# camillabelponer/dealii-slod

Measured on AMD Instinct MI355X. Metric: SLOD patches/sec (basis built), 2D Poisson H=1/32 n_sub=8 oversampling 2, higher is better.
Workload: dtype f64; 1 GPU; C2: 2D Poisson SLOD, H=1/32, n_sub=8, oversampling=2, D1e4 coefficient (contrast 10000), 1024 patches on rank 0 (ensemble of 1 realisations, contiguous patch blocks); patches_per_gpu=1024, parallelism=patch-sharded x1

## Files before the change

dealii-slod_amd/csrc/slod_api.cpp:

```cpp
#include "slod_host.h"

#include <algorithm>
#include <cmath>
#include <cstdio>
#include <cstdlib>
#include <cstring>
#include <string>
#include <vector>

namespace
{
  struct PatchGeom
  {
    int cx, cy, x0, y0, mx, my;
    int side_domain[4];
  };
}

std::string &slod_create_error()
{
  static thread_local std::string e;
  return e;
}

struct slod_plan
{
  slod_handle               *h = nullptr;
  size_t                     n = 0;
  std::vector<SlodPatchDesc> desc;
  SlodPatchDesc             *d_desc = nullptr;
  SlodPatchDesc             *d_desc_bal = nullptr;
  int                        m_max = 0, L_max = 0, nc_max = 0, nb_max = 0, nn_max = 0, nf_max = 0;
  int                        nb_buf = 0;
  size_t                     stride = 0, out_size = 0;
  size_t                     chunk = 0;
  double                    *ws_st = nullptr, *ws_v = nullptr, *ws_x = nullptr, *ws_m = nullptr;
  double                    *ws_z = nullptr;
  double                    *ws_x_alloc = nullptr;
  size_t                     guard = 0;
  size_t                     st_stride = 0, v_stride = 0, x_stride = 0;
  int32_t                   *d_status = nullptr;
  SlodPatchDiag             *d_pdiag  = nullptr;
  SlodSolveChoice            choice;
  std::vector<hipEvent_t>    ev;
  size_t                     n_chunks = 0;
  int                        depth = 1;
  size_t                     n_exec = 0;
  bool                       ran = false;
  struct AltWs
  {
    double  *ws_st = nullptr, *ws_v = nullptr, *ws_x_alloc = nullptr, *ws_x = nullptr, *ws_z = nullptr, *ws_m = nullptr;
    int32_t *d_status = nullptr;
  } alt;
  int         overlap = 1;
  hipStream_t istream[2] = {nullptr, nullptr};
  hipEvent_t  fork_ev = nullptr, done_ev[2] = {nullptr, nullptr};
  bool        inflight[2] = {false, false};
  bool                       uniform_stride = true;
  std::vector<char>          prob_used;
// ... 122 lines not shown
    a.coef_stride = (size_t)h->NE * h->NE * 4;
    a.NE          = h->NE;
    a.n_sub       = h->cfg.n_subdivisions;
    a.quirk       = h->cfg.projection_quirk;
#ifdef SLOD_ENABLE_DIAG
    if (const char *dg = std::getenv("SLOD_DIAG"))
      a.diag = std::atoi(dg);
#endif
    const double H = 1.0 / (double)h->N, hh = H / (double)h->cfg.n_subdivisions;
    a.scale     = hh * hh / 4.0;
    a.invH2     = 1.0 / (H * H);
    a.st        = p->ws_st;
    a.st_stride = p->st_stride;
    a.nn_max    = p->nn_max;
    a.vinv      = p->ws_v;
    a.v_stride  = p->v_stride;
    a.m_max     = p->m_max;
    a.L_max     = p->L_max;
    a.xs        = p->ws_x;
    a.zs        = p->ws_z ? p->ws_z : p->ws_x;
    a.x_stride  = p->x_stride;
    a.nc_max    = p->nc_max;
    a.ms        = p->ws_m;
    a.m_fused   = 0;
    a.nb_buf    = p->nb_buf;
    a.nf_max    = p->nf_max;
    a.fuse_select = 0;
    a.fuse_assemble = 0;
    a.basis     = d_basis;
    a.premult   = d_premult;
    a.status    = p->d_status;
    a.pdiag     = p->d_pdiag;
    if (slot == 1)
      {
        a.st     = p->alt.ws_st;
        a.vinv   = p->alt.ws_v;
        a.xs     = p->alt.ws_x;
        a.zs     = p->alt.ws_z ? p->alt.ws_z : p->alt.ws_x;
        a.ms     = p->alt.ws_m;
        a.status = p->alt.d_status;
      }
    return a;
  }
}

namespace
{
  hipError_t launch_range(slod_plan *p, size_t first, int cnt, double *d_basis, double *d_premult, hipStream_t st,
                          hipEvent_t *ev, bool balanced, int slot = 0)
  {
    const int      s = p->h->cfg.spacedim;
    SlodKernelArgs a = make_args(p, first, d_basis, d_premult, balanced, slot);
    hipError_t     e = ev ? hipEventRecord(ev[0], st) : hipSuccess;
    if (e == hipSuccess && !p->choice.fuse_assemble)
      e = slod_launch_assemble(s, a, cnt, st);
    if (e == hipSuccess && ev)
      e = hipEventRecord(ev[1], st);
    if (e == hipSuccess)
      e = slod_launch_solve(s, p->choice, a, cnt, st);
    if (e == hipSuccess && ev)
      e = hipEventRecord(ev[2], st);
    if (e == hipSuccess && !a.fuse_select)
// ... 273 lines not shown
      return fail(h, SLOD_ERR_UNSUPPORTED, "slod_plan_create: more than 112 dofs per grid line");
    }
  if (p->nc_max > 64)
    {
      slod_plan_destroy(p);
      return fail(h, SLOD_ERR_UNSUPPORTED, "slod_plan_create: more than 64 coarse dofs per patch");
    }
  p->nb_buf = std::min(p->nb_max, std::max(s == 1 ? 96 : 80, p->nc_max + 16));
  if (p->nb_buf > 160)
    {
      slod_plan_destroy(p);
      return fail(h, SLOD_ERR_UNSUPPORTED, "slod_plan_create: boundary-trace buffer beyond the selection kernel's 160 rows");
    }
  if (!slod_choose_solver(s, n_sub, p->m_max, p->L_max, p->nc_max, p->nb_buf, p->nf_max, n, slod_read_tuning(), &p->choice))
    {
      slod_plan_destroy(p);
      return fail(h, SLOD_ERR_UNSUPPORTED, "slod_plan_create: patch does not fit the 160 KB LDS of any solver kernel");
    }
  p->nn_max    = (p->nn_max + 31) & ~31;
  p->st_stride = (size_t)9 * s * s * p->nn_max;
  p->v_stride  = p->choice.v_patch_elems ? p->choice.v_patch_elems : (size_t)p->L_max * p->choice.v_line_elems;
  p->x_stride  = (size_t)p->L_max * p->m_max * p->nc_max;
  const bool   own_z = p->choice.kind == SLOD_K_TW;
  const size_t per_patch = (p->st_stride + p->v_stride + (own_z ? 2 : 1) * p->x_stride) * sizeof(double);
  size_t budget_mb = 24 * 1024;
  {
    size_t free_b = 0, total_b = 0;
    if (hipMemGetInfo(&free_b, &total_b) == hipSuccess)
      {
        const size_t free_mb = free_b / (1024 * 1024);
        budget_mb = std::min(std::max<size_t>(budget_mb, free_mb * 6 / 10), std::max<size_t>(64, free_mb * 8 / 10));
      }
  }
  if (const char *env = std::getenv("SLOD_WORKSPACE_MB"))
    budget_mb = (size_t)std::max(1L, std::atol(env));
  p->chunk = std::max<size_t>(1, std::min<size_t>(n, budget_mb * 1024 * 1024 / per_patch));
  ok = true;
  p->guard = (size_t)24 * p->nc_max + 64;
  const size_t st_slack = (size_t)4 * p->nn_max;
  auto free_ws = [&]() {
    for (double **q : {&p->ws_st, &p->ws_v, &p->ws_x_alloc, &p->ws_z, &p->ws_m})
      if (*q)
        {
          (void)hipFree(*q);
          *q = nullptr;
        }
    p->ws_x = nullptr;
  };
  for (;;)
    {
      bool w = ok;
      w      = w && hipMalloc((void **)&p->ws_st, (p->chunk * p->st_stride + st_slack) * sizeof(double)) == hipSuccess;
      w      = w && hipMalloc((void **)&p->ws_v, std::max<size_t>(1, p->chunk * p->v_stride) * sizeof(double)) == hipSuccess;
      w      = w && hipMalloc((void **)&p->ws_x_alloc, (p->chunk * p->x_stride + 2 * p->guard) * sizeof(double)) == hipSuccess;
      if (own_z)
        w = w && hipMalloc((void **)&p->ws_z, (p->chunk * p->x_stride + p->guard) * sizeof(double)) == hipSuccess;
      w = w && hipMalloc((void **)&p->ws_m, p->chunk * (size_t)p->nc_max * p->nc_max * sizeof(double)) == hipSuccess;
      if (w || !ok || p->chunk == 1)
        {
          ok = w;
          break;
        }
      (void)hipGetLastError();
      free_ws();
      p->chunk = (p->chunk + 1) / 2;
    }
  ok      = ok && hipMemset(p->ws_st, 0, (p->chunk * p->st_stride + st_slack) * sizeof(double)) == hipSuccess;
  ok      = ok && hipMemset(p->ws_x_alloc, 0, (p->chunk * p->x_stride + 2 * p->guard) * sizeof(double)) == hipSuccess;
  p->ws_x = p->ws_x_alloc ? p->ws_x_alloc + p->guard : nullptr;
  if (own_z)
    ok = ok && hipMemset(p->ws_z, 0, (p->chunk * p->x_stride + p->guard) * sizeof(double)) == hipSuccess;
  ok       = ok && hipMalloc((void **)&p->d_status, sizeof(int32_t)) == hipSuccess;
  ok       = ok && hipMalloc((void **)&p->d_pdiag, n * (size_t)s * sizeof(SlodPatchDiag)) == hipSuccess;
  ok       = ok && hipMemset(p->d_pdiag, 0, n * (size_t)s * sizeof(SlodPatchDiag)) == hipSuccess;
  ok = ok && hipMemset(p->d_status, 0, sizeof(int32_t)) == hipSuccess;
  p->n_chunks = (n + p->chunk - 1) / p->chunk;
  p->ev.assign(4 * p->n_chunks, nullptr);
  for (auto &ev : p->ev)
    ok = ok && hipEventCreate(&ev) == hipSuccess;
  if (!ok)
// ... 102 lines not shown
    return SLOD_ERR_ARGUMENT;
  slod_handle *h = p->h;
  if (p->n == 0 || depth == p->overlap)
    return SLOD_OK;
  (void)hipSetDevice(h->cfg.device);
  (void)hipDeviceSynchronize();
  if (depth == 1)
    {
      p->overlap = 1;
      return SLOD_OK;
    }
  if (p->n_chunks != 1)
    return fail(h, SLOD_ERR_STATE, "slod_plan_set_overlap: the plan runs in several workspace chunks (they de-phase by themselves)");
  const bool own_z = p->ws_z != nullptr;
  const size_t st_slack = (size_t)4 * p->nn_max;
  bool ok = true;
  if (!p->alt.ws_st)
    {
      ok = ok && hipMalloc((void **)&p->alt.ws_st, (p->chunk * p->st_stride + st_slack) * sizeof(double)) == hipSuccess;
      ok = ok && hipMalloc((void **)&p->alt.ws_v, std::max<size_t>(1, p->chunk * p->v_stride) * sizeof(double)) == hipSuccess;
      ok = ok && hipMalloc((void **)&p->alt.ws_x_alloc, (p->chunk * p->x_stride + 2 * p->guard) * sizeof(double)) == hipSuccess;
      if (own_z)
        ok = ok && hipMalloc((void **)&p->alt.ws_z, (p->chunk * p->x_stride + p->guard) * sizeof(double)) == hipSuccess;
      ok = ok && hipMalloc((void **)&p->alt.ws_m, p->chunk * (size_t)p->nc_max * p->nc_max * sizeof(double)) == hipSuccess;
      ok = ok && hipMalloc((void **)&p->alt.d_status, sizeof(int32_t)) == hipSuccess;
      ok = ok && hipMemset(p->alt.ws_st, 0, (p->chunk * p->st_stride + st_slack) * sizeof(double)) == hipSuccess;
      ok = ok && hipMemset(p->alt.ws_x_alloc, 0, (p->chunk * p->x_stride + 2 * p->guard) * sizeof(double)) == hipSuccess;
      if (own_z)
        ok = ok && hipMemset(p->alt.ws_z, 0, (p->chunk * p->x_stride + p->guard) * sizeof(double)) == hipSuccess;
      ok = ok && hipMemset(p->alt.d_status, 0, sizeof(int32_t)) == hipSuccess;
      p->alt.ws_x = p->alt.ws_x_alloc ? p->alt.ws_x_alloc + p->guard : nullptr;
      for (int k = 0; k < 2 && ok; ++k)
        {
          ok = ok && hipStreamCreateWithFlags(&p->istream[k], hipStreamNonBlocking) == hipSuccess;
          ok = ok && hipEventCreateWithFlags(&p->done_ev[k], hipEventDisableTiming) == hipSuccess;
        }
      ok = ok && hipEventCreateWithFlags(&p->fork_ev, hipEventDisableTiming) == hipSuccess;
    }
  if (!ok)
    return hip_fail(h, hipGetLastError(), "slod_plan_set_overlap: device allocation");
  p->overlap = 2;
  p->n_exec  = 0;
  return SLOD_OK;
}

int slod_plan_join(slod_plan *p, void *hip_stream)
{
// ... 502 lines not shown
```

dealii-slod_amd/csrc/slod_device.h:

```cpp
#ifndef SLOD_DEVICE_H
#define SLOD_DEVICE_H

#include <hip/hip_runtime.h>
#include <stddef.h>
#include <stdint.h>

struct SlodPatchDesc
{
  int32_t  ox, oy;
  int32_t  nx, ny;
  int32_t  mx, my;
  int32_t  ccx, ccy;
  int32_t  flags;
  int32_t  m, L;
  int32_t  n_c, n_b;
  int32_t  prob;
  uint32_t plan_index;
  uint64_t out_off;
};

enum : int32_t
{
  SLOD_F_LOD        = 1 << 4,
  SLOD_F_TRANSPOSED = 1 << 5
};

#ifdef SLOD_ENABLE_DIAG
#define SLOD_DG(A, mask) ((A).diag & (mask))
#else
#define SLOD_DG(A, mask) 0
#endif

struct SlodPatchDiag
{
  int32_t path;
  int32_t n_cut;
  int32_t n_dropped;
  int32_t sweeps;
  double  dinf;
  double  sigma_max, sigma_min;
};

// ... 4 lines not shown
  const double        *coef1;
  size_t               coef_stride;
  int32_t              NE;
  int32_t              n_sub;
  int32_t              quirk;
  int32_t              diag;
  int32_t              debug;
  double               scale;
  double               invH2;
  double *st;
  size_t  st_stride;
  int32_t nn_max;
  double *vinv;
  size_t  v_stride;
  int32_t m_max;
  int32_t L_max;
  int32_t nv;
  double *xs;
  double *zs;
  size_t  x_stride;
  int32_t nc_max;
  double *ms;
  int32_t m_fused;
  int32_t nb_buf;
  int32_t nf_max;
  int32_t fuse_select;
  int32_t fuse_assemble;
  double  *basis;
  double  *premult;
  int32_t *status;
  SlodPatchDiag *pdiag;
};

enum SlodSolverKind : int32_t
{
  SLOD_K_MF   = 1,
  SLOD_K_TW   = 2,
  SLOD_K_WS   = 3,
  SLOD_K_COOP = 4,
  SLOD_K_ND   = 5
};

struct SlodTuning
{
  int solver = 0;
  int fuse_select = 1, fuse_assemble = 1, fuse_m = 0;
  int twisted = -1;
  int balance = 1;
  int debug = 0;
};
struct SlodSolveChoice
{
  int    kind = 0;
  size_t lds  = 0;
  int    fuse_select = 0, fuse_assemble = 0, m_fused = 0, twisted = 0, debug = 0;
  int    v_line_pad = 0;
  size_t v_line_elems = 0;
  int    nv = 0;
  size_t v_patch_elems = 0;
};
SlodTuning slod_read_tuning();
bool       slod_choose_solver(int S, int n_sub, int m_max, int L_max, int nc_max, int nb_buf, int nf_max, size_t n_patches,
                              const SlodTuning &t, SlodSolveChoice *out);

hipError_t slod_launch_assemble(int S, const SlodKernelArgs &a, int n_patches, hipStream_t st);
hipError_t slod_launch_solve(int S, const SlodSolveChoice &c, SlodKernelArgs &a, int n_patches, hipStream_t st);
hipError_t slod_launch_solve_mf(int S, const SlodKernelArgs &a, int n_patches, size_t lds, hipStream_t st);
hipError_t slod_launch_solve_tw(int S, const SlodKernelArgs &a, int n_patches, size_t lds, hipStream_t st);
hipError_t slod_launch_solve_ws(int S, const SlodKernelArgs &a, int n_patches, size_t lds, hipStream_t st);
hipError_t slod_launch_solve_coop(int S, int twisted, const SlodKernelArgs &a, int n_patches, hipStream_t st);
hipError_t slod_launch_solve_nd(const SlodKernelArgs &a, int n_patches, size_t lds, hipStream_t st);
int        slod_solve_nd_cell(int S, int n_sub, int m_max, int L_max);
size_t     slod_solve_nd_scratch(int nv, int m_max, int L_max, int nc_max);
size_t     slod_solve_nd_lds_bytes(int nv, int m_max, int nc_max);
hipError_t slod_launch_select(int S, const SlodKernelArgs &a, int n_patches, int nb_max,
                              int nf_max, hipStream_t st);
size_t     slod_solve_lds_bytes(int S, int m_max, int nc_max, int twisted);
size_t     slod_solve_ws_lds_bytes(int S, int m_max, int nc_max);
size_t     slod_solve_tw_lds_bytes(int S, int m_max, int nc_max);
size_t     slod_solve_mf_lds_bytes(int S, int m_max, int nc_max);
int        slod_solve_ws_tile(int m_max);
int        slod_solve_mf_tiles(int S, int m_max);
size_t     slod_select_lds_bytes(int S, int nb_max, int nc_max, int nf_max);

#endif
```

dealii-slod_amd/csrc/slod_dispatch.cpp:

```cpp
#include "slod_device.h"

#include <cstdlib>
#include <cstring>

SlodTuning slod_read_tuning()
{
  SlodTuning t;
  if (const char *sel = getenv("SLOD_SOLVE"))
    t.solver = !strcmp(sel, "mf") ? SLOD_K_MF : !strcmp(sel, "tw") ? SLOD_K_TW : !strcmp(sel, "ws") ? SLOD_K_WS :
               !strcmp(sel, "coop") ? SLOD_K_COOP : !strcmp(sel, "nd") ? SLOD_K_ND : 0;
  if (const char *e = getenv("SLOD_FUSE_SELECT"))
    t.fuse_select = atoi(e) ? 1 : 0;
  if (const char *e = getenv("SLOD_FUSE_ASSEMBLE"))
    t.fuse_assemble = atoi(e) ? 1 : 0;
  if (const char *e = getenv("SLOD_FUSE_M"))
    t.fuse_m = atoi(e) ? 1 : 0;
  if (const char *e = getenv("SLOD_TWISTED"))
    t.twisted = atoi(e) ? 1 : 0;
  if (const char *e = getenv("SLOD_BALANCE"))
    t.balance = atoi(e) ? 1 : 0;
  if (const char *e = getenv("SLOD_DEBUG"))
    t.debug = atoi(e) ? 1 : 0;
  return t;
}
// ... 22 lines not shown
      c.v_patch_elems = slod_solve_nd_scratch(nd_nv, m_max, L_max, nc_max);
      c.fuse_assemble = t.fuse_assemble ? 1 : 0;
      c.fuse_select   = 0;
    }
  else if (mf_fits && (t.solver == SLOD_K_MF || (t.solver == 0 && !tw_fits && !ws_fits)))
    {
      c.kind          = SLOD_K_MF;
      c.lds           = slod_solve_mf_lds_bytes(S, m_max, nc_max);
      c.v_line_pad    = 16 * slod_solve_mf_tiles(S, m_max);
      c.v_line_elems  = (size_t)c.v_line_pad * c.v_line_pad;
      c.fuse_assemble = (S == 1 && t.fuse_assemble) ? 1 : 0;
      c.fuse_select   = (S == 1 && t.fuse_select && lds_sel <= lds_max) ? 1 : 0;
      if (c.fuse_select && lds_sel > c.lds)
        c.lds = lds_sel;
    }
  else if (want(SLOD_K_TW) && tw_fits)
    {
      c.kind          = SLOD_K_TW;
      c.lds           = slod_solve_tw_lds_bytes(S, m_max, nc_max);
      c.v_line_pad    = 8 * wt;
      c.v_line_elems  = (size_t)64 * wt * wt;
      c.fuse_assemble = (S == 1 && t.fuse_assemble) ? 1 : 0;
      c.fuse_select = (S == 1 && t.fuse_select && lds_sel <= 64 * 1024) ? 1 : 0;
      if (c.fuse_select && lds_sel > c.lds)
        c.lds = lds_sel;
    }
  else if ((want(SLOD_K_WS) || t.solver == SLOD_K_TW) && ws_fits &&
           slod_solve_ws_lds_bytes(S, m_max, nc_max) <= lds_max)
    {
      c.kind       = SLOD_K_WS;
      c.lds        = slod_solve_ws_lds_bytes(S, m_max, nc_max);
      c.v_line_pad = 8 * wt;
      c.v_line_elems = (size_t)c.v_line_pad * c.v_line_pad;
      c.m_fused = (t.fuse_m && nc_max * nc_max <= 192 * 4) ? 1 : 0;
    }
  else if (t.solver == 0 || t.solver == SLOD_K_COOP || !ws_fits)
    {
      int tw = t.twisted >= 0 ? t.twisted : (n_patches < 3 * 256 ? 1 : 0);
      if (slod_solve_lds_bytes(S, m_max, nc_max, tw) > lds_max)
        tw = 0;
      if (slod_solve_lds_bytes(S, m_max, nc_max, tw) > lds_max || (m_max + 15) / 16 > 7)
        return false;
      c.kind       = SLOD_K_COOP;
      c.twisted    = tw;
      c.lds        = slod_solve_lds_bytes(S, m_max, nc_max, tw);
      c.v_line_pad = m_max;
      c.v_line_elems = (size_t)m_max * m_max;
    }
  else
    return false;
  if (!c.fuse_select && lds_sel > lds_max)
    return false;
  *out = c;
  return true;
}

hipError_t slod_launch_solve(int S, const SlodSolveChoice &c, SlodKernelArgs &a, int n_patches, hipStream_t st)
{
  a.m_fused       = c.m_fused;
  a.fuse_select   = c.fuse_select;
  a.fuse_assemble = c.fuse_assemble;
  a.debug         = c.debug;
  switch (c.kind)
    {
      case SLOD_K_MF:
        return slod_launch_solve_mf(S, a, n_patches, c.lds, st);
      case SLOD_K_TW:
        return slod_launch_solve_tw(S, a, n_patches, c.lds, st);
      case SLOD_K_WS:
        return slod_launch_solve_ws(S, a, n_patches, c.lds, st);
      case SLOD_K_COOP:
        return slod_launch_solve_coop(S, c.twisted, a, n_patches, st);
      case SLOD_K_ND:
        a.nv = c.nv;
        return slod_launch_solve_nd(a, n_patches, c.lds, st);
      default:
        return hipErrorInvalidValue;
    }
}
```

dealii-slod_amd/csrc/slod_select.hip:

```cpp
#include "slod_select.hip.h"

namespace
{
  template <int S>
  __global__ __launch_bounds__(256, S == 1 ? 1 : 2) void k_select(const SlodKernelArgs A, int nb_max, int nf_max)
  {
    extern __shared__ __attribute__((aligned(16))) double smem[];
    select_patch<S, true>(A, nb_max, nf_max, blockIdx.x, smem);
  }
}

size_t slod_select_lds_bytes(int , int nb_max, int nc_max, int nf_max)
{
  const size_t bd = (size_t)nb_max * nc_max > (size_t)nf_max ? (size_t)nb_max * nc_max : (size_t)nf_max;
  const size_t n  = (size_t)nc_max * (nc_max + 1) + (size_t)nc_max * nc_max + bd + 5 * (size_t)nc_max + 8 +
                   2 * (size_t)(nb_max > 160 ? nb_max : 160);
  return n * sizeof(double) + (5 * (size_t)nc_max + 4) * sizeof(int);
}

hipError_t slod_launch_select(int S, const SlodKernelArgs &a, int n_patches, int nb_max, int nf_max,
                              hipStream_t st)
{
  const size_t lds = slod_select_lds_bytes(S, nb_max, a.nc_max, nf_max);
  hipError_t   e;
  if (S == 1)
    {
      e = hipFuncSetAttribute(reinterpret_cast<const void *>(k_select<1>),
                              hipFuncAttributeMaxDynamicSharedMemorySize, (int)lds);
      if (e != hipSuccess)
        return e;
      hipLaunchKernelGGL(k_select<1>, dim3(n_patches), dim3(256), lds, st, a, nb_max, nf_max);
// ... 12 lines not shown
```

dealii-slod_amd/csrc/slod_select.hip.h:

```cpp
#ifndef SLOD_SELECT_HIP_H
#define SLOD_SELECT_HIP_H
#include "slod_common.hip.h"

namespace
{

  template <int S, bool OWN = false>
  __device__ __forceinline__ void select_patch(const SlodKernelArgs &A, const int nb_max, const int nf_max,
                                               const int patch, double *smem)
  {
    const SlodPatchDesc d   = A.desc[patch];
    const int           tid = threadIdx.x;
    const int           nc = d.n_c, nb = d.n_b, n = A.n_sub;
    const int           ncm = A.nc_max, ldm = ncm + 1;
    const int           mm = A.m_max, ncs = A.nc_max;
    const bool          tr  = (d.flags & SLOD_F_TRANSPOSED) != 0;
    const bool          lod = (d.flags & SLOD_F_LOD) != 0;
    const int           npx = d.nx + 1, nn = npx * (d.ny + 1), nf = S * nn;

    double *Ms   = smem;
    double *Vj   = Ms + ncm * ldm;
    double *BD   = Vj + ncm * ncm;
    double *phis = BD;
    double *sig  = BD + max(nb_max * ncm, nf_max);
    double *utg  = sig + ncm;
    double *gam  = utg + ncm;
    double *cvec = gam + ncm;
    double *rowk = cvec + ncm;
    double *red  = rowk + ncm;
    const int vst = max(nb_max, 160);
    double *vcol = red + 8;
    int    *colk = reinterpret_cast<int *>(vcol + 2 * vst);
// ... 38 lines not shown
        cell_of_col(d, c / S, kx, ky);
        colk[c]       = kx;
        colk[ncm + c] = ky;
      }
    __syncthreads();

    const bool stamping = (SLOD_DG(A, (1 << 20))) && tid == 0 && A.nc_max * A.nc_max >= 12;
    double    *msd      = A.ms + (size_t)patch * A.nc_max * A.nc_max;
    double     tph[3]   = {0.0, 0.0, 0.0};
    double     tlast    = stamping ? (double)wall_clock64() : 0.0;
    auto       stamp    = [&](int i) {
      if (stamping)
        msd[i] = tlast = (double)wall_clock64();
    };
    auto tacc = [&](int i) {
      if (stamping)
        {
          const double now = (double)wall_clock64();
          tph[i] += now - tlast;
          tlast = now;
        }
    };

    if (A.m_fused)
      {
        const double *mg = A.ms + (size_t)patch * A.nc_max * A.nc_max;
        for (int idx = tid; idx < nc * nc; idx += 256)
          Ms[(idx / nc) * ldm + (idx % nc)] = mg[idx];
      }
    for (int idx = tid; idx < ((SLOD_DG(A, 64)) || A.m_fused ? 0 : nc * (nc + 1) / 2); idx += 256)
      {
        int a = (int)((2.0f * nc + 1.0f - sqrtf((2.0f * nc + 1.0f) * (2.0f * nc + 1.0f) - 8.0f * idx)) * 0.5f);
        a     = min(max(a, 0), nc - 1);
        while (a > 0 && a * (2 * nc - a + 1) / 2 > idx)
          --a;
        while (a + 1 < nc && (a + 1) * (2 * nc - a) / 2 <= idx)
          ++a;
        const int b  = a + idx - a * (2 * nc - a + 1) / 2;
        const int kx = colk[a], ky = colk[ncm + a];
        double    acc = 0.0;
        if (S == 1 || !A.quirk)
          {
            const int ca = a % S;
            for (int jy0 = 0; jy0 <= n; jy0 += 3)
              for (int jx0 = 0; jx0 <= n; jx0 += 9)
                {
                  double xv[3][9];
#pragma unroll
                  for (int ry = 0; ry < 3; ++ry)
                    {
                      const int iy  = ky * n + jy0 + ry;
                      const int iyc = min(max(iy, 1), d.ny - 1);
#pragma unroll
// ... 1046 lines not shown
```

dealii-slod_amd/csrc/slod_solve_tw.hip:

```cpp
#include <type_traits>
#include "slod_assemble.hip.h"
#include "slod_select.hip.h"

namespace
{
  template <int T, int S>
  __global__ __launch_bounds__(256, ws_min_waves(T)) void k_solve_tw(const SlodKernelArgs A)
  {
    extern __shared__ __attribute__((aligned(16))) double smem[];
    const SlodPatchDesc d = A.desc[blockIdx.x];
    constexpr int       W = 2 * S - 1, BW = 2 * W + 1, MP = 8 * T;
    constexpr int       BWP = BW + 1, BROWS = MP + 2 * W, bsz = (BROWS * BWP + 1) & ~1;
    const int           tid = threadIdx.x, wave = __builtin_amdgcn_readfirstlane(tid >> 6);
    int                 lane = tid & 63;
    const int           chain = wave & 1;
    const bool          is_gj = wave < 2;
    const int           m = d.m, L = d.L, nc = d.n_c, n = A.n_sub;
    const int           mm = A.m_max, ncs = (A.nc_max + 1) & ~1, ncg = A.nc_max;
    const bool          tr  = (d.flags & SLOD_F_TRANSPOSED) != 0;
    const int           npx = d.nx + 1;
    const int           chsz = MP * ncs + MP + 6 * bsz;

    double *cb   = smem + chain * chsz;
    double *Rb   = cb;
    double *rowb = Rb + MP * ncs;
    double *Tf   = rowb + MP;
    double *Tn0  = Tf + bsz;
    double *Tn1  = Tn0 + bsz;
    double *Bc0  = Tn1 + bsz;
    double *Bc1  = Bc0 + bsz;
    auto    Bbuf = [&](double *base, int stp) { return base + ((stp + 3) % 3) * bsz; };
    double *ocb  = smem + (1 - chain) * chsz;
    int    *colk = reinterpret_cast<int *>(smem + 2 * chsz);
    int *perm = colk + 2 * A.nc_max + chain * 3 * A.nc_max, *inv = perm + A.nc_max, *act = inv + A.nc_max;
    int *operm = colk + 2 * A.nc_max + (1 - chain) * 3 * A.nc_max, *oinv = operm + A.nc_max, *oact = oinv + A.nc_max;
    (void)operm;

    const double *st    = A.st + (size_t)blockIdx.x * A.st_stride;
    double       *vg    = A.vinv + (size_t)blockIdx.x * A.v_stride;
    double       *xg    = A.xs + (size_t)blockIdx.x * A.x_stride;
    double       *zg    = A.zs + (size_t)blockIdx.x * A.x_stride;
    const size_t  vline = (size_t)64 * T * T, xline = (size_t)mm * ncg;
    auto load_A = [&](const double *vl, int ti, double (&dst)[MP / 4]) __attribute__((always_inline)) {
      const int     row = min(16 * ti + (lane & 15), MP - 1);
      const int     rt = row / T, rr = row - rt * T, kq = lane >> 4;
      const double *base = vl + (rt * 8 + kq) * (T * T) + rr * T;
#pragma unroll
      for (int g = 0; g < 2; ++g)
#pragma unroll
        for (int kr = 0; kr < T; ++kr)
          dst[g * T + kr] = base[g * 4 * T * T + kr];
    };
    auto brow = [&](int kk) { return T * ((lane >> 4) + 4 * (kk / T)) + kk % T; };

    const int mid = L / 2;
    auto mid_tile = [&](int ti) __attribute__((always_inline)) {
      const double *vl = vg + (size_t)mid * vline;
      double       *xl = xg + (size_t)mid * xline;
      const int     tiles_j = (nc + 15) >> 4;
      double        av[MP / 4];
      load_A(vl, ti, av);
      for (int tj = 0; tj < tiles_j; tj += 2)
        {
          double4_t     acc0 = {0.0, 0.0, 0.0, 0.0}, acc1 = {0.0, 0.0, 0.0, 0.0};
          const double *bp  = smem + 16 * tj + (lane & 15);
          const bool    two = tj + 1 < tiles_j;
#pragma unroll
          for (int kk = 0; kk < MP / 4; ++kk)
            {
              acc0 = __builtin_amdgcn_mfma_f64_16x16x4f64(av[kk], bp[brow(kk) * ncs], acc0, 0, 0, 0);
              if (two)
                acc1 = __builtin_amdgcn_mfma_f64_16x16x4f64(av[kk], bp[brow(kk) * ncs + 16], acc1, 0, 0, 0);
            }
#pragma unroll
          for (int r = 0; r < 4; ++r)
            {
              const int row = 16 * ti + (lane >> 4) + 4 * r, col = 16 * tj + (lane & 15);
              if (row < m && col < nc)
                xl[row * ncg + col] = acc0[r];
              if (two && row < m && col + 16 < nc)
                xl[row * ncg + col + 16] = acc1[r];
            }
        }
    };
    const int n0 = mid, n1 = L - 1 - mid, nstp = n0 > n1 ? n0 : n1;
    const int nmy = chain == 0 ? n0 : n1;
    const int dl  = chain == 0 ? 1 : -1;
    auto      line_of = [&](int c, int t) { return c == 0 ? t : L - 1 - t; };

    if ((SLOD_DG(A, (1 << 20))) && tid == 0)
      {
        A.ms[(size_t)blockIdx.x * A.nc_max * A.nc_max] = (double)wall_clock64();
        if (A.nc_max * A.nc_max >= 16)
          {
            A.ms[(size_t)blockIdx.x * A.nc_max * A.nc_max + 12] = (double)__builtin_amdgcn_s_getreg((31 << 11) | 4);
            A.ms[(size_t)blockIdx.x * A.nc_max * A.nc_max + 13] = (double)__builtin_amdgcn_s_getreg((31 << 11) | 20);
          }
      }
    if ((SLOD_DG(A, (1 << 20))) && lane == 0 && A.nc_max * A.nc_max >= 24)
      A.ms[(size_t)blockIdx.x * A.nc_max * A.nc_max + 20 + wave] = (double)__builtin_amdgcn_s_getreg((31 << 11) | 4);
    auto tstamp = [&](int k) {
      if ((SLOD_DG(A, (1 << 20))) && tid == 0 && A.nc_max * A.nc_max >= 48)
        A.ms[(size_t)blockIdx.x * A.nc_max * A.nc_max + 32 + k] = (double)wall_clock64();
    };
    tstamp(0);
    if (S == 1 && A.fuse_assemble)
      {
        for (int node = tid; node < npx * (d.ny + 1); node += 256)
          assemble_node<S>(A, d, blockIdx.x, node);
        __syncthreads();
      }
    for (int idx = tid; idx < 2 * chsz; idx += 256)
      smem[idx] = 0.0;
    for (int c = tid; c < nc; c += 256)
      {
        int kx, ky;
        cell_of_col(d, c / S, kx, ky);
        colk[c]            = kx;
        colk[A.nc_max + c] = ky;
      }
    __syncthreads();
    {
      auto first_step = [&](int ch, int c) {
        const int kq = tr ? colk[c] : colk[A.nc_max + c];
        const int a  = ch == 0 ? kq * n - 1 : L - (kq + 1) * n;
        return a > 0 ? a : 0;
      };
      for (int idx = tid; idx < 2 * nc; idx += 256)
        {
          const int ch = idx / nc, c = idx - ch * nc, a = first_step(ch, c);
          int       rank = 0;
          for (int c2 = 0; c2 < nc; ++c2)
            {
              const int a2 = first_step(ch, c2);
              rank += (a2 < a || (a2 == a && c2 < c)) ? 1 : 0;
            }
// ... 7 lines not shown
      for (int idx = t0; idx < m * BW; idx += nt)
        {
          const int i = idx / BW, oi = idx - i * BW, o = oi - W;
          if (Tdst)
            Tdst[(i + W) * BWP + oi] = with_T ? coupling<S>(st, A.nn_max, npx, tr, m, line, i, 0, o) : 0.0;
          if (Bdst)
            Bdst[(i + W) * BWP + oi] = coupling<S>(st, A.nn_max, npx, tr, m, line, i, dl, o);
        }
    };
    auto put_step = [&](int stp, int t0, int nt) __attribute__((always_inline)) {
      if (stp >= nmy)
        return;
      put_bands(line_of(chain, stp + 1), (stp & 1) ? Tn1 : Tn0, !(chain == 1 && stp + 1 == nmy), nullptr, t0, nt);
      put_bands(line_of(chain, stp), nullptr, true, Bbuf(Bc0, stp), t0, nt);
    };
    {
      const int t0 = (wave >> 1) * 64 + lane;
      put_bands(line_of(chain, 0), Tf, true, nullptr, t0, 128);
      put_step(0, t0, 128);
      put_step(1, t0, 128);
    }
    __syncthreads();
    tstamp(1);

    if (is_gj)
      {
        __builtin_amdgcn_s_setprio(3);
        int    gy = lane >> 3, gx = lane & 7;
        double a[T][T];
        auto dpp_from_prev = [](double x) {
          const int lo = __builtin_amdgcn_update_dpp(0, __double2loint(x), 0x111, 0xf, 0xf, true);
          const int hi = __builtin_amdgcn_update_dpp(0, __double2hiint(x), 0x111, 0xf, 0xf, true);
          return __hiloint2double(hi, lo);
        };
        auto dpp_from_next = [](double x) {
          const int lo = __builtin_amdgcn_update_dpp(0, __double2loint(x), 0x101, 0xf, 0xf, true);
          const int hi = __builtin_amdgcn_update_dpp(0, __double2hiint(x), 0x101, 0xf, 0xf, true);
          return __hiloint2double(hi, lo);
        };
        auto next_S_w1 = [&](const double *Tsrc, const double *Bl) __attribute__((always_inline)) {
          const double *cbp = Bl + (T * gx) * BWP + 2;
          const double *dbp = Bl + (T * gy) * BWP + 2;
          double        cb[T][3], db[T][3];
#pragma unroll
          for (int tb = 0; tb < T; ++tb)
#pragma unroll
// ... 241 lines not shown
            if (A.nc_max * A.nc_max >= 52)
              for (int k = 0; k < 2; ++k)
                A.ms[(size_t)blockIdx.x * A.nc_max * A.nc_max + 48 + k] = acc_p[k];
          }
        tstamp(2);
        if (chain == 1)
          store_tile(vg + (size_t)mid * vline, 1.0);
        __syncthreads();
        if (chain == 0)
          {
            const double *w1 = vg + (size_t)mid * vline + (gy * 8 + gx) * (T * T);
#pragma unroll
            for (int ta = 0; ta < T; ++ta)
#pragma unroll
              for (int tb = 0; tb < T; ++tb)
                a[ta][tb] += w1[ta * T + tb];
            sweep();
            store_tile(vg + (size_t)mid * vline, -1.0);
          }
        if (bad != 0 && lane == 0 && !SLOD_DG(A, -1))
          atomicOr(A.status, 1);
        __builtin_amdgcn_s_setprio(0);
        __syncthreads();
        if (!(SLOD_DG(A, 8)))
          for (int ti = wave; 16 * ti < m; ti += 4)
            mid_tile(ti);
        __syncthreads();
      }
    else
      {
        auto build_R = [&](int line, const double *Bprev, const double *zprev, int zstride, bool with_F, bool add, int ncols,
                           const int *cmap, const int *zmap, const int *zact, int tlim, bool zlds) __attribute__((always_inline)) {
          if (SLOD_DG(A, 2))
            return;
          constexpr int CP = 2;
          const int     g = lane >> 3, cq = lane & 7;
          const double *zp = zprev ? zprev : zg;
          for (int r0 = 0; r0 < ncols; r0 += 8 * CP)
            {
              double win[CP][T + 2 * W];
              int    kxn[CP], kyn[CP], cc[CP];
              bool   valid[CP];
#pragma unroll
              for (int k = 0; k < CP; ++k)
                {
                  const int r  = r0 + 8 * k + cq;
                  valid[k]     = r < ncols;
                  const int rc = valid[k] ? r : 0;
                  const int c = cmap ? cmap[rc] : rc, zc = zmap ? zmap[rc] : rc;
                  const bool zok = valid[k] && zprev && zact[zc] <= tlim;
// ... 140 lines not shown
                    {
                      const int row = 16 * ti + (lane >> 4) + 4 * r, col = lane & 15;
                      if (row < m && col < ncols)
                        {
                          xl[row * ncols + col] = acc0[r];
                          Rb[row * ncs + col]   = acc0[r];
                        }
                      if (two && row < m && col + 16 < ncols)
                        {
                          xl[row * ncols + col + 16] = acc1[r];
                          Rb[row * ncs + col + 16]   = acc1[r];
                        }
                    }
                  if (ti + 1 < TI)
                    {
#pragma unroll
                      for (int kk = 0; kk < MP / 4; ++kk)
                        av[kk] = an[kk];
                    }
                }
            }
          __builtin_amdgcn_fence(__ATOMIC_RELEASE, "wavefront");
          __builtin_amdgcn_wave_barrier();
        };
        constexpr int NBQ = (MP * BW + 63) / 64;
        double        tq[NBQ], bq_[NBQ];
        auto fetch_step = [&](int stp) __attribute__((always_inline)) {
          const bool on = stp < nmy;
          const int  lT = line_of(chain, stp + 1), lB = line_of(chain, stp);
          const bool with_T = !(chain == 1 && stp + 1 == nmy);
#pragma unroll
          for (int q = 0; q < NBQ; ++q)
            {
              const int  idx = lane + 64 * q, i = idx / BW, oi = idx - i * BW, o = oi - W, j = i + o;
              const int  pi = i / S, ci = i - pi * S, pj = j / S, cj = j - pj * S, dp = pj - pi;
              const bool ok = on && idx < m * BW && j >= 0 && j < m && dp >= -1 && dp <= 1;
              const int ixT = tr ? lT + 1 : pi + 1, iyT = tr ? pi + 1 : lT + 1;
              const int ixB = tr ? lB + 1 : pi + 1, iyB = tr ? pi + 1 : lB + 1;
              const int dirT = (tr ? dp : 0) * 3 + (tr ? 0 : dp) + 4;
              const int dirB = ((tr ? dp : dl) + 1) * 3 + (tr ? dl : dp) + 1;
              const double vT = st[ok ? (size_t)((dirT * S + ci) * S + cj) * A.nn_max + ixT + iyT * npx : 0];
              const double vB = st[ok ? (size_t)((dirB * S + ci) * S + cj) * A.nn_max + ixB + iyB * npx : 0];
              tq[q]  = (ok && with_T) ? vT : 0.0;
              bq_[q] = ok ? vB : 0.0;
            }
        };
// ... 70 lines not shown
          for (int k = 0; k < 4; ++k)
            A.ms[(size_t)blockIdx.x * A.nc_max * A.nc_max + 44 + k] = acc_h[k];
        if (nmy == nstp && nmy > 0)
          fwd_step(nstp - 1);
        __syncthreads();
        if (chain == 0)
          {
            const double *B0 = Bbuf(Bc0, n0 - 1);
            double       *ob = ocb + MP * ncs + MP + 3 * bsz;
            const double *B1 = Bbuf(ob, n1 - 1);
            int na0 = 0, na1 = 0;
            while (na0 < nc && act[na0] <= n0 - 1)
              ++na0;
            while (na1 < nc && oact[na1] <= n1 - 1)
              ++na1;
            build_R(mid, B0, n0 > 0 ? zg + (size_t)(mid - 1) * xline : nullptr, na0, true, false, nc, nullptr, inv, act,
                    n0 - 1, false);
            __builtin_amdgcn_wave_barrier();
            if (n1 > 0)
              build_R(mid, B1, zg + (size_t)(mid + 1) * xline, na1, false, true, nc, nullptr, oinv, oact, n1 - 1, false);
            __builtin_amdgcn_fence(__ATOMIC_RELEASE, "wavefront");
            __builtin_amdgcn_wave_barrier();
          }
        __syncthreads();
        if (!(SLOD_DG(A, 8)))
          for (int ti = wave; 16 * ti < m; ti += 4)
            mid_tile(ti);
        __syncthreads();
      }

    tstamp(3);
    {
      const int t128 = (wave >> 1) * 64 + lane, w2 = wave >> 1;
      const int tiles_i = (m + 15) >> 4, tiles_j = (nc + 15) >> 4;
      constexpr int NBV = (MP * BW + 127) / 128;
      double        bv[NBV];
      auto fetch_B = [&](int line) __attribute__((always_inline)) {
#pragma unroll
        for (int q = 0; q < NBV; ++q)
          {
            const int idx = t128 + 128 * q, i = idx / BW, o = idx - i * BW - W;
            bv[q] = (idx < m * BW) ? coupling<S>(st, A.nn_max, npx, tr, m, line, i, dl, o) : 0.0;
          }
      };
      auto store_B = [&](double *Bdst) __attribute__((always_inline)) {
#pragma unroll
        for (int q = 0; q < NBV; ++q)
          {
            const int idx = t128 + 128 * q, i = idx / BW, oi = idx - i * BW;
            if (idx < m * BW)
              Bdst[(i + W) * BWP + oi] = bv[q];
// ... 221 lines not shown
                  for (int r = 0; r < 4; ++r)
                    {
                      const int row = 16 * ti + (lane >> 4) + 4 * r;
                      if (row < m && col < nc)
                        xl[row * ncg + col] = zl[r] - acc[r];
                    }
                }
              if (t > 0)
                store_B(((t - 1) & 1) ? Bc1 : Bc0);
            }
        }
      };
      if (keepb)
        backward(std::true_type{});
      else
        backward(std::false_type{});
    }
    const bool stamp = (SLOD_DG(A, (1 << 20))) && tid == 0;
    if (stamp)
      A.ms[(size_t)blockIdx.x * A.nc_max * A.nc_max + 1] = (double)wall_clock64();
    if (S == 1 && A.fuse_select)
      {
        __syncthreads();
        select_patch<S>(A, A.nb_buf, A.nf_max, blockIdx.x, smem);
        if (stamp)
          A.ms[(size_t)blockIdx.x * A.nc_max * A.nc_max + 2] = (double)wall_clock64();
      }
  }

}

size_t slod_solve_tw_lds_bytes(int S, int m_max, int nc_max)
{
  const int    T = slod_solve_ws_tile(m_max), W = 2 * S - 1, BW = 2 * W + 1, MP = 8 * T;
  const int    ncs = (nc_max + 1) & ~1, bsz = ((MP + 2 * W) * (BW + 1) + 1) & ~1;
  (void)m_max;
  const size_t chsz = (size_t)MP * ncs + MP + 6 * (size_t)bsz;
  return ((2 * chsz * sizeof(double) + 8 * (size_t)nc_max * sizeof(int)) + 15) & ~(size_t)15;
}

template <int T, int S>
static hipError_t launch_tw_TS(const SlodKernelArgs &a, int n_patches, size_t lds, hipStream_t st)
{
  const void *fn = reinterpret_cast<const void *>(k_solve_tw<T, S>);
  hipError_t  e  = hipFuncSetAttribute(fn, hipFuncAttributeMaxDynamicSharedMemorySize, (int)lds);
  if (e != hipSuccess)
    return e;
  if (a.debug)
    {
      int nb = 0;
      (void)hipOccupancyMaxActiveBlocksPerMultiprocessor(&nb, fn, 256, lds);
      fprintf(stderr, "[slod] k_solve_tw<%d,%d>: %d patches, lds %zu B, occupancy %d blocks/CU\n", T, S, n_patches,
              lds, nb);
    }
  hipLaunchKernelGGL((k_solve_tw<T, S>), dim3(n_patches), dim3(256), lds, st, a);
  return hipGetLastError();
}

template <int S>
static hipError_t launch_tw_S(const SlodKernelArgs &a, int n_patches, size_t lds, hipStream_t st)
{
  switch (slod_solve_ws_tile(a.m_max))
    {
      case 2:
        return launch_tw_TS<2, S>(a, n_patches, lds, st);
      case 3:
        return launch_tw_TS<3, S>(a, n_patches, lds, st);
      case 4:
        return launch_tw_TS<4, S>(a, n_patches, lds, st);
      case 5:
        return launch_tw_TS<5, S>(a, n_patches, lds, st);
      case 6:
        return launch_tw_TS<6, S>(a, n_patches, lds, st);
      case 8:
        return launch_tw_TS<8, S>(a, n_patches, lds, st);
      case 10:
// ... 15 lines not shown
```

Before: 1.043 million patches/s.

## Accumulate the coarse Gram matrix M inside the twisted solver sweeps

Fuses the computation of the per-patch coarse matrix M into the twisted-factorisation solve kernel. It accumulates partial products with f64 MFMA during both chain sweeps and the middle-line tile, and writes the result to a new per-patch mt buffer with a validity flag. The selection step then reads this precomputed M instead of recomputing the nc(nc+1)/2 dot products. This makes fuse_m the default, at the cost of extra LDS, extra registers in the sweeps, and more workspace memory, and it is enabled only when LDS occupancy is unchanged.

```diff
diff --git a/dealii-slod_amd/csrc/slod_api.cpp b/dealii-slod_amd/csrc/slod_api.cpp
--- a/dealii-slod_amd/csrc/slod_api.cpp
+++ b/dealii-slod_amd/csrc/slod_api.cpp
@@ -34,7 +34,8 @@
   int                        nb_buf = 0;
   size_t                     stride = 0, out_size = 0;
   size_t                     chunk = 0;
-  double                    *ws_st = nullptr, *ws_v = nullptr, *ws_x = nullptr, *ws_m = nullptr;
+  double                    *ws_st = nullptr, *ws_v = nullptr, *ws_x = nullptr;
+  double                    *ws_m = nullptr;
   double                    *ws_z = nullptr;
   double                    *ws_x_alloc = nullptr;
   size_t                     guard = 0;
@@ -203,7 +204,9 @@
     a.x_stride  = p->x_stride;
     a.nc_max    = p->nc_max;
     a.ms        = p->ws_m;
+    a.mt        = p->ws_m + p->chunk * (size_t)p->nc_max * p->nc_max;
     a.m_fused   = 0;
+    a.m_tw      = 0;
     a.nb_buf    = p->nb_buf;
     a.nf_max    = p->nf_max;
     a.fuse_select = 0;
@@ -219,6 +222,7 @@
         a.xs     = p->alt.ws_x;
         a.zs     = p->alt.ws_z ? p->alt.ws_z : p->alt.ws_x;
         a.ms     = p->alt.ws_m;
+        a.mt     = p->alt.ws_m + p->chunk * (size_t)p->nc_max * p->nc_max;
         a.status = p->alt.d_status;
       }
     return a;
@@ -538,7 +542,8 @@
   p->v_stride  = p->choice.v_patch_elems ? p->choice.v_patch_elems : (size_t)p->L_max * p->choice.v_line_elems;
   p->x_stride  = (size_t)p->L_max * p->m_max * p->nc_max;
   const bool   own_z = p->choice.kind == SLOD_K_TW;
-  const size_t per_patch = (p->st_stride + p->v_stride + (own_z ? 2 : 1) * p->x_stride) * sizeof(double);
+  const size_t per_patch =
+    (p->st_stride + p->v_stride + (own_z ? 2 : 1) * p->x_stride + 2 * (size_t)p->nc_max * p->nc_max + 1) * sizeof(double);
   size_t budget_mb = 24 * 1024;
   {
     size_t free_b = 0, total_b = 0;
@@ -571,7 +576,7 @@
       w      = w && hipMalloc((void **)&p->ws_x_alloc, (p->chunk * p->x_stride + 2 * p->guard) * sizeof(double)) == hipSuccess;
       if (own_z)
         w = w && hipMalloc((void **)&p->ws_z, (p->chunk * p->x_stride + p->guard) * sizeof(double)) == hipSuccess;
-      w = w && hipMalloc((void **)&p->ws_m, p->chunk * (size_t)p->nc_max * p->nc_max * sizeof(double)) == hipSuccess;
+      w = w && hipMalloc((void **)&p->ws_m, p->chunk * (2 * (size_t)p->nc_max * p->nc_max + 1) * sizeof(double)) == hipSuccess;
       if (w || !ok || p->chunk == 1)
         {
           ok = w;
@@ -720,7 +725,7 @@
       ok = ok && hipMalloc((void **)&p->alt.ws_x_alloc, (p->chunk * p->x_stride + 2 * p->guard) * sizeof(double)) == hipSuccess;
       if (own_z)
         ok = ok && hipMalloc((void **)&p->alt.ws_z, (p->chunk * p->x_stride + p->guard) * sizeof(double)) == hipSuccess;
-      ok = ok && hipMalloc((void **)&p->alt.ws_m, p->chunk * (size_t)p->nc_max * p->nc_max * sizeof(double)) == hipSuccess;
+      ok = ok && hipMalloc((void **)&p->alt.ws_m, p->chunk * (2 * (size_t)p->nc_max * p->nc_max + 1) * sizeof(double)) == hipSuccess;
       ok = ok && hipMalloc((void **)&p->alt.d_status, sizeof(int32_t)) == hipSuccess;
       ok = ok && hipMemset(p->alt.ws_st, 0, (p->chunk * p->st_stride + st_slack) * sizeof(double)) == hipSuccess;
       ok = ok && hipMemset(p->alt.ws_x_alloc, 0, (p->chunk * p->x_stride + 2 * p->guard) * sizeof(double)) == hipSuccess;
diff --git a/dealii-slod_amd/csrc/slod_device.h b/dealii-slod_amd/csrc/slod_device.h
--- a/dealii-slod_amd/csrc/slod_device.h
+++ b/dealii-slod_amd/csrc/slod_device.h
@@ -18,6 +18,8 @@
   uint32_t plan_index;
   uint64_t out_off;
 };
+
+__host__ __device__ inline size_t slod_mt_stride(int nc_max) { return (size_t)nc_max * nc_max + 1; }
 
 enum : int32_t
 {
@@ -68,6 +70,8 @@
   int32_t nc_max;
   double *ms;
   int32_t m_fused;
+  double *mt;
+  int32_t m_tw;
   int32_t nb_buf;
   int32_t nf_max;
   int32_t fuse_select;
@@ -90,7 +94,7 @@
 struct SlodTuning
 {
   int solver = 0;
-  int fuse_select = 1, fuse_assemble = 1, fuse_m = 0;
+  int fuse_select = 1, fuse_assemble = 1, fuse_m = -1;
   int twisted = -1;
   int balance = 1;
   int debug = 0;
@@ -99,7 +103,7 @@
 {
   int    kind = 0;
   size_t lds  = 0;
-  int    fuse_select = 0, fuse_assemble = 0, m_fused = 0, twisted = 0, debug = 0;
+  int    fuse_select = 0, fuse_assemble = 0, m_fused = 0, m_tw = 0, twisted = 0, debug = 0;
   int    v_line_pad = 0;
   size_t v_line_elems = 0;
   int    nv = 0;
@@ -123,7 +127,7 @@
                               int nf_max, hipStream_t st);
 size_t     slod_solve_lds_bytes(int S, int m_max, int nc_max, int twisted);
 size_t     slod_solve_ws_lds_bytes(int S, int m_max, int nc_max);
-size_t     slod_solve_tw_lds_bytes(int S, int m_max, int nc_max);
+size_t     slod_solve_tw_lds_bytes(int S, int m_max, int nc_max, bool with_m = false);
 size_t     slod_solve_mf_lds_bytes(int S, int m_max, int nc_max);
 int        slod_solve_ws_tile(int m_max);
 int        slod_solve_mf_tiles(int S, int m_max);
diff --git a/dealii-slod_amd/csrc/slod_dispatch.cpp b/dealii-slod_amd/csrc/slod_dispatch.cpp
--- a/dealii-slod_amd/csrc/slod_dispatch.cpp
+++ b/dealii-slod_amd/csrc/slod_dispatch.cpp
@@ -1,5 +1,6 @@
 #include "slod_device.h"
 
+#include <algorithm>
 #include <cstdlib>
 #include <cstring>
 
@@ -68,6 +69,16 @@
       c.v_line_elems  = (size_t)64 * wt * wt;
       c.fuse_assemble = (S == 1 && t.fuse_assemble) ? 1 : 0;
       c.fuse_select = (S == 1 && t.fuse_select && lds_sel <= 64 * 1024) ? 1 : 0;
+      if (S == 1 && t.fuse_m != 0 && nc_max <= 32 && 8 * wt <= 48)
+        {
+          const size_t sel    = c.fuse_select ? lds_sel : 0;
+          const size_t with_m = std::max(slod_solve_tw_lds_bytes(S, m_max, nc_max, true), sel);
+          if (std::min<size_t>(4, lds_max / with_m) == std::min<size_t>(4, lds_max / std::max(c.lds, sel)))
+            {
+              c.m_tw = 1;
+              c.lds  = slod_solve_tw_lds_bytes(S, m_max, nc_max, true);
+            }
+        }
       if (c.fuse_select && lds_sel > c.lds)
         c.lds = lds_sel;
     }
@@ -78,7 +89,7 @@
       c.lds        = slod_solve_ws_lds_bytes(S, m_max, nc_max);
       c.v_line_pad = 8 * wt;
       c.v_line_elems = (size_t)c.v_line_pad * c.v_line_pad;
-      c.m_fused = (t.fuse_m && nc_max * nc_max <= 192 * 4) ? 1 : 0;
+      c.m_fused = (t.fuse_m > 0 && nc_max * nc_max <= 192 * 4) ? 1 : 0;
     }
   else if (t.solver == 0 || t.solver == SLOD_K_COOP || !ws_fits)
     {
@@ -104,6 +115,7 @@
 hipError_t slod_launch_solve(int S, const SlodSolveChoice &c, SlodKernelArgs &a, int n_patches, hipStream_t st)
 {
   a.m_fused       = c.m_fused;
+  a.m_tw          = c.m_tw;
   a.fuse_select   = c.fuse_select;
   a.fuse_assemble = c.fuse_assemble;
   a.debug         = c.debug;
diff --git a/dealii-slod_amd/csrc/slod_select.hip b/dealii-slod_amd/csrc/slod_select.hip
--- a/dealii-slod_amd/csrc/slod_select.hip
+++ b/dealii-slod_amd/csrc/slod_select.hip
@@ -6,7 +6,9 @@
   __global__ __launch_bounds__(256, S == 1 ? 1 : 2) void k_select(const SlodKernelArgs A, int nb_max, int nf_max)
   {
     extern __shared__ __attribute__((aligned(16))) double smem[];
-    select_patch<S, true>(A, nb_max, nf_max, blockIdx.x, smem);
+    const double *mt = A.m_tw ? A.mt + (size_t)blockIdx.x * slod_mt_stride(A.nc_max) : nullptr;
+    select_patch<S, true>(A, nb_max, nf_max, blockIdx.x, smem,
+                          (mt && mt[(size_t)A.nc_max * A.nc_max] != 0.0) ? mt : nullptr);
   }
 }
 
diff --git a/dealii-slod_amd/csrc/slod_select.hip.h b/dealii-slod_amd/csrc/slod_select.hip.h
--- a/dealii-slod_amd/csrc/slod_select.hip.h
+++ b/dealii-slod_amd/csrc/slod_select.hip.h
@@ -7,7 +7,7 @@
 
   template <int S, bool OWN = false>
   __device__ __forceinline__ void select_patch(const SlodKernelArgs &A, const int nb_max, const int nf_max,
-                                               const int patch, double *smem)
+                                               const int patch, double *smem, const double *mpre = nullptr)
   {
     const SlodPatchDesc d   = A.desc[patch];
     const int           tid = threadIdx.x;
@@ -92,13 +92,14 @@
         }
     };
 
-    if (A.m_fused)
+    const bool m_given = mpre != nullptr || A.m_fused;
+    if (m_given)
       {
-        const double *mg = A.ms + (size_t)patch * A.nc_max * A.nc_max;
+        const double *mg = mpre ? mpre : A.ms + (size_t)patch * A.nc_max * A.nc_max;
         for (int idx = tid; idx < nc * nc; idx += 256)
           Ms[(idx / nc) * ldm + (idx % nc)] = mg[idx];
       }
-    for (int idx = tid; idx < ((SLOD_DG(A, 64)) || A.m_fused ? 0 : nc * (nc + 1) / 2); idx += 256)
+    for (int idx = tid; idx < ((SLOD_DG(A, 64)) || m_given ? 0 : nc * (nc + 1) / 2); idx += 256)
       {
         int a = (int)((2.0f * nc + 1.0f - sqrtf((2.0f * nc + 1.0f) * (2.0f * nc + 1.0f) - 8.0f * idx)) * 0.5f);
         a     = min(max(a, 0), nc - 1);
diff --git a/dealii-slod_amd/csrc/slod_solve_tw.hip b/dealii-slod_amd/csrc/slod_solve_tw.hip
--- a/dealii-slod_amd/csrc/slod_solve_tw.hip
+++ b/dealii-slod_amd/csrc/slod_solve_tw.hip
@@ -35,6 +35,17 @@
     int *perm = colk + 2 * A.nc_max + chain * 3 * A.nc_max, *inv = perm + A.nc_max, *act = inv + A.nc_max;
     int *operm = colk + 2 * A.nc_max + (1 - chain) * 3 * A.nc_max, *oinv = operm + A.nc_max, *oact = oinv + A.nc_max;
     (void)operm;
+    double *mtile = smem + 2 * chsz + 4 * A.nc_max;
+    double *mfull = smem + chsz;
+    bool    mfuse = false;
+    auto nafin = [&](int ch) {
+      const int *ac = colk + 2 * A.nc_max + ch * 3 * A.nc_max + 2 * A.nc_max;
+      const int  nl = ch == 0 ? L / 2 : L - 1 - L / 2;
+      int        na = 0;
+      for (int k = 0; k < nc; ++k)
+        na += ac[k] <= nl - 1 ? 1 : 0;
+      return na;
+    };
 
     const double *st    = A.st + (size_t)blockIdx.x * A.st_stride;
     double       *vg    = A.vinv + (size_t)blockIdx.x * A.v_stride;
@@ -54,7 +65,8 @@
     auto brow = [&](int kk) { return T * ((lane >> 4) + 4 * (kk / T)) + kk % T; };
 
     const int mid = L / 2;
-    auto mid_tile = [&](int ti) __attribute__((always_inline)) {
+    double4_t pm[3] = {{0.0, 0.0, 0.0, 0.0}, {0.0, 0.0, 0.0, 0.0}, {0.0, 0.0, 0.0, 0.0}};
+    auto mid_tile = [&](int ti, bool with_m) __attribute__((always_inline)) {
       const double *vl = vg + (size_t)mid * vline;
       double       *xl = xg + (size_t)mid * xline;
       const int     tiles_j = (nc + 15) >> 4;
@@ -81,7 +93,73 @@
               if (two && row < m && col + 16 < nc)
                 xl[row * ncg + col + 16] = acc1[r];
             }
+          if (with_m)
+            {
+              double ra[2][4];
+#pragma unroll
+              for (int it = 0; it < 2; ++it)
+#pragma unroll
+                for (int r = 0; r < 4; ++r)
+                  {
+                    const int  k = 16 * ti + (lane >> 4) + 4 * r, i = 16 * it + (lane & 15);
+                    const bool ok = k < m && i < nc;
+                    const double v = smem[ok ? k * ncs + i : 0];
+                    ra[it][r] = ok ? v : 0.0;
+                  }
+#pragma unroll
+              for (int r = 0; r < 4; ++r)
+                {
+                  pm[0] = __builtin_amdgcn_mfma_f64_16x16x4f64(ra[0][r], acc0[r], pm[0], 0, 0, 0);
+                  if (two)
+                    {
+                      pm[1] = __builtin_amdgcn_mfma_f64_16x16x4f64(ra[0][r], acc1[r], pm[1], 0, 0, 0);
+                      pm[2] = __builtin_amdgcn_mfma_f64_16x16x4f64(ra[1][r], acc1[r], pm[2], 0, 0, 0);
+                    }
+                }
+            }
         }
+    };
+    auto mid_phase = [&]() __attribute__((always_inline)) {
+      if (!(SLOD_DG(A, 8)))
+        for (int ti = wave; 16 * ti < m; ti += 4)
+          mid_tile(ti, mfuse);
+      if (mfuse)
+        {
+          const int nw   = min((m + 15) >> 4, 4);
+          double   *mtg  = A.mt + (size_t)blockIdx.x * slod_mt_stride(A.nc_max);
+          auto      turn = [&](bool last) __attribute__((always_inline)) {
+#pragma unroll
+            for (int q = 0; q < 3; ++q)
+#pragma unroll
+              for (int r = 0; r < 4; ++r)
+                {
+                  const int i = 16 * (q == 2 ? 1 : 0) + (lane >> 4) + 4 * r, j = 16 * (q == 0 ? 0 : 1) + (lane & 15);
+                  if (i <= j && j < nc)
+                    {
+                      const double v = mfull[i * nc + j] + pm[q][r];
+                      if (last)
+                        {
+                          mtg[i * nc + j] = v * A.invH2;
+                          mtg[j * nc + i] = v * A.invH2;
+                        }
+                      else
+                        {
+                          mfull[i * nc + j] = v;
+                          mfull[j * nc + i] = v;
+                        }
+                    }
+                }
+          };
+          for (int w = 0; w + 1 < nw; ++w)
+            {
+              if (wave == w)
+                turn(false);
+              __syncthreads();
+            }
+          if (wave == nw - 1)
+            turn(true);
+        }
+      __syncthreads();
     };
     const int n0 = mid, n1 = L - 1 - mid, nstp = n0 > n1 ? n0 : n1;
     const int nmy = chain == 0 ? n0 : n1;
@@ -112,6 +190,9 @@
       }
     for (int idx = tid; idx < 2 * chsz; idx += 256)
       smem[idx] = 0.0;
+    if (A.m_tw)
+      for (int idx = tid; idx < 2 * 256; idx += 256)
+        mtile[idx] = 0.0;
     for (int c = tid; c < nc; c += 256)
       {
         int kx, ky;
@@ -165,6 +246,17 @@
     }
     __syncthreads();
     tstamp(1);
+    mfuse = S == 1 && A.m_tw && (MP + 15) / 16 <= 3 && nc <= 32 &&
+                 nc * nc <= MP * ncs + MP + 3 * bsz && !(SLOD_DG(A, 8));
+    int na_end[2] = {0, 0};
+    if (mfuse)
+      {
+        na_end[0] = __builtin_amdgcn_readfirstlane(nafin(0));
+        na_end[1] = __builtin_amdgcn_readfirstlane(nafin(1));
+        mfuse     = na_end[0] <= 16 && na_end[1] <= 16;
+      }
+    if (A.m_tw && tid == 0)
+      A.mt[(size_t)blockIdx.x * slod_mt_stride(A.nc_max) + (size_t)A.nc_max * A.nc_max] = mfuse ? 1.0 : 0.0;
 
     if (is_gj)
       {
@@ -452,10 +544,7 @@
           atomicOr(A.status, 1);
         __builtin_amdgcn_s_setprio(0);
         __syncthreads();
-        if (!(SLOD_DG(A, 8)))
-          for (int ti = wave; 16 * ti < m; ti += 4)
-            mid_tile(ti);
-        __syncthreads();
+        mid_phase();
       }
     else
       {
@@ -642,6 +731,23 @@
             }
           __builtin_amdgcn_fence(__ATOMIC_RELEASE, "wavefront");
           __builtin_amdgcn_wave_barrier();
+          if (mfuse)
+            {
+              __builtin_amdgcn_fence(__ATOMIC_ACQUIRE, "wavefront");
+              double   *mtc = mtile + chain * 256 + (lane >> 4) * 16 + (lane & 15);
+              double4_t macc;
+#pragma unroll
+              for (int r = 0; r < 4; ++r)
+                macc[r] = mtc[64 * r];
+#pragma unroll
+              for (int kk = 0; kk < MP / 4; ++kk)
+                macc = __builtin_amdgcn_mfma_f64_16x16x4f64(bq[0][kk], bp[brow(kk) * ncs], macc, 0, 0, 0);
+#pragma unroll
+              for (int r = 0; r < 4; ++r)
+                mtc[64 * r] = macc[r];
+              __builtin_amdgcn_fence(__ATOMIC_RELEASE, "wavefront");
+              __builtin_amdgcn_wave_barrier();
+            }
         };
         constexpr int NBQ = (MP * BW + 63) / 64;
         double        tq[NBQ], bq_[NBQ];
@@ -758,11 +864,26 @@
             __builtin_amdgcn_fence(__ATOMIC_RELEASE, "wavefront");
             __builtin_amdgcn_wave_barrier();
           }
+        else if (mfuse)
+          {
+            const int na0 = na_end[0], na1 = na_end[1];
+            for (int idx = lane; idx < nc * nc; idx += 64)
+              {
+                const int a = idx / nc, b = idx - a * nc, lo = min(a, b), hi = max(a, b);
+                double    v = 0.0;
+#pragma unroll
+                for (int ch = 0; ch < 2; ++ch)
+                  {
+                    const int *ci = colk + 2 * A.nc_max + ch * 3 * A.nc_max + A.nc_max;
+                    const int  i0 = ci[lo], j0 = ci[hi];
+                    if (i0 < (ch ? na1 : na0) && j0 < (ch ? na1 : na0))
+                      v += mtile[ch * 256 + i0 * 16 + j0];
+                  }
+                mfull[idx] = v;
+              }
+          }
         __syncthreads();
-        if (!(SLOD_DG(A, 8)))
-          for (int ti = wave; 16 * ti < m; ti += 4)
-            mid_tile(ti);
-        __syncthreads();
+        mid_phase();
       }
 
     tstamp(3);
@@ -1030,7 +1151,8 @@
     if (S == 1 && A.fuse_select)
       {
         __syncthreads();
-        select_patch<S>(A, A.nb_buf, A.nf_max, blockIdx.x, smem);
+        select_patch<S>(A, A.nb_buf, A.nf_max, blockIdx.x, smem,
+                        mfuse ? A.mt + (size_t)blockIdx.x * slod_mt_stride(A.nc_max) : nullptr);
         if (stamp)
           A.ms[(size_t)blockIdx.x * A.nc_max * A.nc_max + 2] = (double)wall_clock64();
       }
@@ -1038,13 +1160,14 @@
 
 }
 
-size_t slod_solve_tw_lds_bytes(int S, int m_max, int nc_max)
+size_t slod_solve_tw_lds_bytes(int S, int m_max, int nc_max, bool with_m)
 {
   const int    T = slod_solve_ws_tile(m_max), W = 2 * S - 1, BW = 2 * W + 1, MP = 8 * T;
   const int    ncs = (nc_max + 1) & ~1, bsz = ((MP + 2 * W) * (BW + 1) + 1) & ~1;
   (void)m_max;
-  const size_t chsz = (size_t)MP * ncs + MP + 6 * (size_t)bsz;
-  return ((2 * chsz * sizeof(double) + 8 * (size_t)nc_max * sizeof(int)) + 15) & ~(size_t)15;
+  const size_t chsz  = (size_t)MP * ncs + MP + 6 * (size_t)bsz;
+  const size_t mtile = with_m ? 2 * 256 * sizeof(double) : 0;
+  return ((2 * chsz * sizeof(double) + 8 * (size_t)nc_max * sizeof(int) + mtile) + 15) & ~(size_t)15;
 }
 
 template <int T, int S>
@@ -1058,8 +1181,8 @@
     {
       int nb = 0;
       (void)hipOccupancyMaxActiveBlocksPerMultiprocessor(&nb, fn, 256, lds);
-      fprintf(stderr, "[slod] k_solve_tw<%d,%d>: %d patches, lds %zu B, occupancy %d blocks/CU\n", T, S, n_patches,
-              lds, nb);
+      fprintf(stderr, "[slod] k_solve_tw<%d,%d>: %d patches, lds %zu B, occupancy %d blocks/CU, M in the sweeps %d\n", T,
+              S, n_patches, lds, nb, a.m_tw);
     }
   hipLaunchKernelGGL((k_solve_tw<T, S>), dim3(n_patches), dim3(256), lds, st, a);
   return hipGetLastError();
```

Result: faster. 1.075 million patches/s, median of 6 (+3.1%).
